# vladiant/CascadeClassifier

Measured on AMD Instinct MI355X. Metric: detection Mwindows/sec (1080p, haarcascade_frontalface) + achieved HBM GB/s, higher is better.
Workload: dtype i32+f32 (f64 stage sums)

## Files before the change

### cascadeclassifier_amd/_lib.py

```python
from __future__ import annotations

import ctypes as C
import os

_HERE = os.path.dirname(os.path.abspath(__file__))
LIB_PATH = os.environ.get("CCAMD_LIB") or os.path.join(_HERE, "lib", "libcascadeclassifier_amd.so")

CC_OK = 0
CC_ERR_INVALID_ARG = -1
CC_ERR_NO_DEVICE = -2
CC_ERR_HIP = -3
CC_ERR_IO = -4
CC_ERR_PARSE = -5
CC_ERR_UNSUPPORTED = -6
CC_ERR_BUFFER_TOO_SMALL = -7
CC_ERR_OUT_OF_RANGE = -8

CC_FEATURE_HAAR, CC_FEATURE_LBP, CC_FEATURE_HOG = 0, 1, 2
CC_PIX_GRAY8, CC_PIX_BGR8, CC_PIX_BGRA8, CC_PIX_RGB8, CC_PIX_RGBA8, CC_PIX_RGB8_PLANAR = 0, 1, 2, 3, 4, 5
CC_HAAR_BASIC, CC_HAAR_CORE, CC_HAAR_ALL = 0, 1, 2


class CascadeError(RuntimeError):

# ... 86 lines not shown
                                              _vp, C.POINTER(_i)]),
    "cc_detect_multiscale_levels_fmt": (_i, [_vp, _vp, _i, _i, _sz, _i, C.POINTER(DetectParams), _vp, _vp, _vp, _i,
                                             C.POINTER(_i)]),
    "cc_to_gray_u8": (_i, [_i, _vp, _i, _i, _i, _sz, _vp, _sz]),
    "cc_detect_multiscale_levels": (_i, [_vp, _vp, _i, _i, _sz, C.POINTER(DetectParams), _vp, _vp, _vp, _i, C.POINTER(_i)]),
    "cc_detect_raw": (_i, [_vp, _vp, _i, _i, _sz, C.POINTER(DetectParams), _vp, _i, C.POINTER(_i)]),
    "cc_detect_debug_windows": (_i, [_vp, _vp, _i, _i, _sz, C.POINTER(DetectParams), _vp, _vp, _vp, C.c_int64,
                                     C.POINTER(C.c_int64)]),
    "cc_scale_plan": (_i, [_i, _i, _i, _i, C.POINTER(DetectParams), _vp, _i, C.POINTER(_i)]),
    "cc_detector_specialize": (_i, [_vp, _i]),
    "cc_detector_specialize_async": (_i, [_vp, _i]),
    "cc_detector_specialized_stages": (_i, [_vp]),
    "cc_cascade_compile_specialized": (_i, [_vp, _i, C.c_char_p, C.POINTER(C.c_size_t)]),
    "cc_detector_set_profiling": (_i, [_vp, _i]),
    "cc_detector_graph_active": (_i, [_vp]),
    "cc_detector_graph_captures": (C.c_int64, [_vp]),
    "cc_detector_get_timings": (_i, [_vp, C.POINTER(DetectorTimings), _i]),
    "cc_detector_candidate_capacity": (_i, [_vp]),
    "cc_integral_u8": (_i, [_i, _vp, _i, _i, _sz, _vp, _vp, _vp]),
    "cc_resize_linear_exact_u8": (_i, [_i, _vp, _i, _i, _sz, _vp, _i, _i, _sz]),
    "cc_debug_stream_dwords": (_i, [_i, _sz, _i, C.POINTER(C.c_uint32)]),
    "cc_debug_division_check": (_i, [_i, C.c_uint64, C.c_uint64, C.POINTER(C.c_uint64)]),
    "cc_debug_vnf_check": (_i, [_i, C.c_uint64, C.c_uint64, C.POINTER(C.c_uint64)]),
    "cc_group_rectangles": (_i, [_vp, _i, _i, _d, _vp, _i, C.POINTER(_i)]),
    "cc_group_rectangles_device": (_i, [_i, _vp, _vp, _i, _i, _d, _vp, _i, _vp, C.POINTER(_i)]),
    "cc_group_rectangles_levels": (_i, [_vp, _vp, _vp, _i, _i, _d, _vp, _vp, _vp, _i, C.POINTER(_i)]),
    "cc_group_rectangles_device_levels": (_i, [_i, _vp, _vp, _vp, _vp, _i, _i, _d, _vp, _vp, _vp, _i, _vp, C.POINTER(_i)]),
    "cc_eval_create": (_i, [_i, _i, _i, _i, _i, _i, _pp]),
    "cc_eval_destroy": (None, [_vp]),
    "cc_eval_num_features": (_i, [_vp]),
    "cc_eval_max_cat_count": (_i, [_vp]),
    "cc_eval_feature_size": (_i, [_vp]),
    "cc_eval_feature_geometry": (_i, [_vp, _i, _vp, _vp, C.POINTER(_i)]),
    "cc_eval_set_image": (_i, [_vp, _vp, _sz, C.c_uint8, _i]),
    "cc_eval_set_images": (_i, [_vp, _vp, _i, _i, _vp]),
    "cc_eval_labels": (C.POINTER(C.c_float), [_vp]),
    "cc_eval_calc": (_i, [_vp, _i, _i, C.POINTER(C.c_float)]),
    "cc_eval_calc_list": (_i, [_vp, _vp, _i, _i, _vp]),
    "cc_eval_calc_batch": (_i, [_vp, _i, _i, _vp, _i, _vp, _i]),
    "cc_eval_calc_batch_device": (_i, [_vp, _i, _i, _vp, _i, _vp, _sz]),
    "cc_eval_calc_batch_sorted": (_i, [_vp, _i, _i, _i, _vp, _vp, _i]),
    "cc_eval_calc_custom_haar": (_i, [_vp, _vp, _i, _i, _vp, _i, _vp]),
    "cc_haar_feature_calc": (_i, [_i, _vp, _i, _i, _vp, _vp, _i, _i, _vp]),
    "cc_eval_get_sample": (_i, [_vp, _i, _vp, _vp, _vp]),
    "cc_eval_hog_feature_geometry": (_i, [_vp, _i, _vp]),
    "cc_eval_get_hog_sample": (_i, [_vp, _i, _vp, _vp]),
# ... 70 lines not shown
```

### cascadeclassifier_amd/csrc/cc_detect.hip

```cpp
#include <hip/hip_runtime.h>

#include <algorithm>

#include "cc_detector.h"

namespace ccamd {

#include "cc_eval_kernel.inc"

__global__ __launch_bounds__(256) void k_stream_dwords(const uint32_t* __restrict__ p, size_t n_words, uint32_t* __restrict__ out) {
  uint32_t acc = 0;
  for (size_t i = (size_t)blockIdx.x * blockDim.x + threadIdx.x; i < n_words; i += (size_t)gridDim.x * blockDim.x) acc += p[i];
  if (acc == 0x9e3779b9u) atomicAdd(out, acc);
  atomicAdd(out + 1 + (threadIdx.x & 15), acc);
}

__device__ __forceinline__ bool visited_by_scan(const unsigned long long* __restrict__ row_mask, int gx) {
  int run = 0;
  int pos = gx - 1;
  while (pos >= 0) {
    const int b = pos & 63;
    const unsigned long long w = row_mask[pos >> 6] << (63 - b);
    const int ones = min(__clzll((long long)~w), b + 1);
    run += ones;
// ... 82 lines not shown
  A.stage_first = d->d_stage_first.p;
  A.stage_ntrees = d->d_stage_ntrees.p;
  A.group_first = d->d_group_first.p;
  A.ngroups = d->n_groups;
  A.dense_from = d->dense_from;
  A.wave_below = d->wave_below;
  A.stop_after = d->stop_after;
  A.split_stumps = d->split_stumps;
  A.early_skip = d->early_skip;
  A.sq_compact = sq_compact;
  A.stage_thr = d->d_stage_thr.p;
  A.masks = d->d_masks[slot].p;
  A.mask_frame_words = P->mask_frame_words;
  A.cands = d->d_cands[slot].p;
  A.cand_count = d->d_counts[slot].p;
  A.cand_cap = d->cand_cap;
  A.stamps = nullptr;
  A.dbg_codes = debug ? d->d_dbg_codes.p : nullptr;
  A.dbg_sums = debug ? d->d_dbg_sums.p : nullptr;
  A.stumps1 = haar ? (const void*)d->d_haar1.p : (const void*)d->d_lbp1.p;
  A.stumps2 = haar ? (const void*)d->d_haar2.p : (const void*)d->d_lbp2.p;
  A.wstumps1 = d->d_haar1w.p ? (const void*)d->d_haar1w.p : A.stumps1;
  A.wstumps2 = d->d_haar2w.p ? (const void*)d->d_haar2w.p : A.stumps2;
  A.gstumps = haar ? (const void*)d->d_haar_g.p : (const void*)d->d_lbp_g.p;
  A.lbp16_all = d->lbp16_all;
  if (!haar && d->d_lbp16.p) A.wstumps2 = d->d_lbp16.p;
  A.trees = d->m.max_nodes_per_tree > 1 ? 1 : 0;
  A.nodes1 = haar ? (const void*)d->d_hnode1.p : (const void*)d->d_lnode1.p;
  A.nodes2 = haar ? (const void*)d->d_hnode2.p : (const void*)d->d_lnode2.p;
  A.tree_root = d->d_tree_root.p;
  A.tree_leaf0 = d->d_tree_leaf0.p;
  A.leaves = d->d_leaves.p;
  return A;
}

int eval_stamp_slots() { return STAMP_SLOTS; }

cc_status launch_eval(cc_detector* d, const Plan* P, int slot, int nchan, bool tilt, int sq_compact, bool debug, unsigned long long* stamps,
                      const EvalLaunch* launches, int n_launches, int nf, hipStream_t st) {
  const bool haar = d->m.feature_type == CC_FEATURE_HAAR;
  EvalArgs A = eval_args(d, P, slot, nchan, tilt, sq_compact, debug);
  A.stamps = stamps;
  for (int i = 0; i < n_launches; i++) {
    const EvalLaunch& L = launches[i];
    if (L.n_tiles == 0) continue;
    A.tiles = L.tiles;
// ... 79 lines not shown
```

### cascadeclassifier_amd/csrc/cc_detector.h

```cpp
#pragma once
#include <atomic>
#include <functional>
#include <future>
#include <map>
#include <memory>
#include <thread>

#include "cc_detect_internal.h"

namespace ccamd {

struct Plan {
  int w = 0, h = 0;
  cc_detect_params p{};
  std::vector<ScaleGeom> geom;
  FrontTables front;
  size_t mask_frame_words = 0;
  long long windows = 0, integral_elems = 0;
  int n_grid_rows = 0;
  struct TileList {
    int n = 0;
    DevBuf<int4> d;
  };
  std::map<std::pair<int, int>, TileList> tiles;
// ... 58 lines not shown

constexpr int kStageSlots = 3;

struct cc_detector {
  Cascade m;
  unsigned long long serial = 0;
  int device = 0;
  int max_batch = 1;
  int pass_capacity = 1;
  OwnStream own_stream;
  hipStream_t stream = nullptr;
  DevBuf<int> d_stage_ntrees, d_stage_first;
  std::vector<int> group_first;
  DevBuf<int> d_group_first;
  int n_groups = 0;
  int dense_from = 0x7fffffff;
  DevBuf<float> d_stage_thr;
  int wave_below = 0;
  int last_call_graph = 0;
  int stop_after = -1;
  int split_stumps = 0;
  DevBuf<HaarStumpDev> d_haar1, d_haar2;
  DevBuf<HaarStumpDev> d_haar1w, d_haar2w;
  DevBuf<HaarStumpDev> d_haar_g;
  DevBuf<LbpStumpDev> d_lbp_g, d_lbp16;
  int lbp16_all = 0;
  DevBuf<LbpStumpDev> d_lbp1, d_lbp2;
  DevBuf<HaarNodeDev> d_hnode1, d_hnode2;
  DevBuf<LbpNodeDev> d_lnode1, d_lnode2;
  DevBuf<int> d_tree_root, d_tree_leaf0;
  DevBuf<float> d_leaves;
  size_t lds = 0;
  std::vector<std::unique_ptr<Plan>> plans;
  DevBuf<uint8_t> d_frames, d_pyr;
  DevBuf<int32_t> d_integ[2], d_hbuf, d_diag, d_tseg;
  OwnStream front_stream;
  OwnEvent front_done[2], eval_done[2], batch_begin;
  bool eval_pending[2] = {false, false};
  int overlap_front = 1;
  SpecModule spec[2];
  int n_spec = 0;
  int last_stamp_tiles = 0;
  int spec_stages = 0;
  int auto_specialize = 0;
  std::thread spec_thread;
  std::atomic<int> spec_bg_state{0};
// ... 99 lines not shown
```

### cascadeclassifier_amd/csrc/cc_eval_kernel.inc

```

#define CC_CONST __attribute__((address_space(4)))
template <class T>
__device__ __forceinline__ const T CC_CONST* as_const_table(const T* p) {
  return (const T CC_CONST*)p;
}
template <class T>
__device__ __forceinline__ T load_record(const T CC_CONST* p) {
  static_assert(sizeof(T) % 4 == 0, "table records are dword multiples");
  T out;
  const int CC_CONST* w = (const int CC_CONST*)p;
  int* o = reinterpret_cast<int*>(&out);
#pragma unroll
  for (unsigned i = 0; i < sizeof(T) / 4; i++) o[i] = w[i];
  return out;
}

constexpr int STAGE_ROWS = 12;
template <int STEP, class Geom>
__device__ __forceinline__ void stage_tile(int32_t* lds, const Geom& G, const int32_t* __restrict__ sum,
                                           const ScaleDev& S, int x0, int y0) {
  const int lane = threadIdx.x & 63, wave = __builtin_amdgcn_readfirstlane(threadIdx.x >> 6);
  const int quads = (G.cols + 3) >> 2;
  const bool right_edge = x0 + quads * 4 - 1 > S.w;
  for (int q0 = 0; q0 < quads; q0 += 64) {
// ... 34 lines not shown
    }
  }
}

struct EvalArgs {
  const int32_t* integ;
  size_t int_frame_elems;
  int nchan;
  int tilt_chan;
  const ScaleDev* sd;
  const int4* tiles;
  int W0, H0;
  int nstages;
  const int* stage_first;
  const int* stage_ntrees;
  const float* stage_thr;
  const int* group_first;
  int ngroups;
  int dense_from;
  const void* stumps1;
  const void* stumps2;
  const void* wstumps1;
  const void* wstumps2;
  const void* gstumps;
  int lbp16_all;
  int trees;
  const void* nodes1;
  const void* nodes2;
  const int* tree_root;
  const int* tree_leaf0;
  const float* leaves;
  int wave_below;
  int early_skip;
  int sq_compact;
  int split_stumps;
  int stop_after;
  unsigned long long* masks;
  size_t mask_frame_words;
  CandRaw* cands;
  int* cand_count;
  int cand_cap;
  int32_t* dbg_codes;
  double* dbg_sums;
  unsigned long long* stamps;
};
constexpr int STAMP_SLOTS = 40;

struct LdsReader {
  const int32_t* b;
  __device__ __forceinline__ int operator()(int ofs) const { return b[ofs]; }
};
struct GlobalReader {
  const int32_t* g;
  unsigned org;
  int pitch;
  __device__ __forceinline__ int operator()(int p) const { return g[org + (unsigned)((p >> 16) * pitch + (p & 0xffff))]; }
};
template <class R>
__device__ __forceinline__ double stump_vote(const R& rd, const HaarStumpDev& sp, float vnf) {
  const int r0 = rd(sp.ofs[0][0]) - rd(sp.ofs[0][1]) - rd(sp.ofs[0][2]) + rd(sp.ofs[0][3]);
  const int r1 = rd(sp.ofs[1][0]) - rd(sp.ofs[1][1]) - rd(sp.ofs[1][2]) + rd(sp.ofs[1][3]);
  float v = sp.w[0] * (float)r0 + sp.w[1] * (float)r1;
  if (sp.nrect == 3) {
    const int r2 = rd(sp.ofs[2][0]) - rd(sp.ofs[2][1]) - rd(sp.ofs[2][2]) + rd(sp.ofs[2][3]);
    v += sp.w[2] * (float)r2;
  }
  v *= vnf;
  return (double)(v < sp.thr ? sp.left : sp.right);
}
template <class R>
__device__ __forceinline__ double stump_vote(const R& rd, const HaarStumpDev CC_CONST* spp, float vnf) {
  return stump_vote(rd, load_record(spp), vnf);
}

struct Lds16Reader {
  const unsigned short* h;
  __device__ __forceinline__ int operator()(int ofs) const { return (int)h[ofs]; }
};
template <bool M16, class R>
__device__ __forceinline__ float lbp_vote_f(const R& rd, const LbpStumpDev& sp) {
  int p[16];
#pragma unroll
  for (int j = 0; j < 16; j++) p[j] = rd(sp.ofs[j]);
  auto cell = [&](int a, int b, int c2, int d) {
    const int v = p[a] - p[b] - p[c2] + p[d];
    return M16 ? (v & 0xffff) : v;
  };
  const int c = cell(5, 6, 9, 10);
  const bool b7 = cell(0, 1, 4, 5) >= c, b6 = cell(1, 2, 5, 6) >= c, b5 = cell(2, 3, 6, 7) >= c;
  const int lo = (cell(6, 7, 10, 11) >= c ? 16 : 0) | (cell(10, 11, 14, 15) >= c ? 8 : 0) | (cell(9, 10, 13, 14) >= c ? 4 : 0) |
                 (cell(8, 9, 12, 13) >= c ? 2 : 0) | (cell(4, 5, 8, 9) >= c ? 1 : 0);
// ... 52 lines not shown

template <int CTRL, int ROW_MASK>
__device__ __forceinline__ int dpp_i32(int v) {
  return __builtin_amdgcn_update_dpp(0, v, CTRL, ROW_MASK, 0xF, false);
}
__device__ __forceinline__ int wave_max_u32(int v) {
  v = max(v, dpp_i32<0xB1, 0xF>(v));
  v = max(v, dpp_i32<0x4E, 0xF>(v));
  v = max(v, dpp_i32<0x141, 0xF>(v));
  v = max(v, dpp_i32<0x140, 0xF>(v));
  v = max(v, dpp_i32<0x142, 0xA>(v));
  v = max(v, dpp_i32<0x143, 0xC>(v));
  return __builtin_amdgcn_readlane(v, 63);
}
__device__ __forceinline__ int wave_sum_u32(int v) {
  v += dpp_i32<0xB1, 0xF>(v);
  v += dpp_i32<0x4E, 0xF>(v);
  v += dpp_i32<0x141, 0xF>(v);
  v += dpp_i32<0x140, 0xF>(v);
  v += dpp_i32<0x142, 0xA>(v);
  v += dpp_i32<0x143, 0xC>(v);
  return __builtin_amdgcn_readlane(v, 63);
}

__device__ __forceinline__ float inv_sqrt_as_float(double nf) {
#ifndef CC_EXACT_SLOW_VNF
  double y = __builtin_amdgcn_rsq(nf);
#pragma unroll
  for (int it = 0; it < 2; it++) {
    const double e = __builtin_fma(-(nf * y), y, 1.0);
    y = __builtin_fma(0.5 * y, e, y);
  }
  const unsigned below = (unsigned)(unsigned long long)__double_as_longlong(y) & 0x1fffffffu;
  if (__builtin_expect(below - 0x0ffffc00u > 0x800u, 1)) return (float)y;
#endif
  return (float)(1. / sqrt(nf));
}

#ifdef CC_SPEC_STAGES
template <int STEP>
__device__ __forceinline__ double spec_stage(int st, int p_lo, int p_hi, const int32_t* b, float vnf);
template <int STEP>
__device__ __forceinline__ void spec_stage0_x2(const int32_t* ba, const int32_t* bb, float vnfa, float vnfb, double& acc_a, double& acc_b);
#endif

template <bool C, class A, class B>
// ... 32 lines not shown
  const ScaleDev& S;
#ifdef CC_SPEC_W0
  static constexpr int W0 = CC_SPEC_W0, H0 = CC_SPEC_H0;
#else
  const int W0 = A.W0, H0 = A.H0;
#endif
  const Geom G{W0, H0};
  double* const s_part = reinterpret_cast<double*>(lds + tile_words_padded(G.words()) * ((HAAR && A.tilt_chan >= 0) ? 2 : 1));
  float* const s_vnf = reinterpret_cast<float*>(s_part + PART_DOUBLES);
  unsigned short* const s_q = reinterpret_cast<unsigned short*>(s_vnf + (HAAR ? TILE_Y * VNF_PITCH : 0));
  int* const s_cnt = reinterpret_cast<int*>(s_q + 2 * TILE_WINDOWS);
  const int frame = blockIdx.y;
  const int32_t* const sum = A.integ + ((size_t)frame * A.nchan + 0) * A.int_frame_elems + S.int_ofs;
  const int lane = threadIdx.x & 63, wave = __builtin_amdgcn_readfirstlane(threadIdx.x >> 6);
  const int half = lane >> 5, cls = lane & 31;
  const int gx0 = T.y * TILE_X, gy0 = T.z * TILE_Y;
  const int skew = (STEP * G.row_stride) & 31;
  const Node* const nodes = reinterpret_cast<const Node*>(STEP == 2 ? A.nodes2 : A.nodes1);
  const Stump CC_CONST* const stumps = as_const_table(reinterpret_cast<const Stump*>(G16 ? A.gstumps : STEP == 2 ? A.stumps2 : A.stumps1));
  const int CC_CONST* const stage_first = as_const_table(A.stage_first);
  const int CC_CONST* const stage_ntrees = as_const_table(A.stage_ntrees);
  const float CC_CONST* const stage_thr = as_const_table(A.stage_thr);
  const int CC_CONST* const group_first = as_const_table(A.group_first);
  const bool dbg = A.dbg_codes != nullptr && frame == 0;

  __device__ __forceinline__ EvalTile(const EvalArgs& A_, int32_t* lds_, const int4 T_, const ScaleDev& S_) : A(A_), lds(lds_), T(T_), S(S_) {}

  __device__ __forceinline__ void stamp(int slot) const {
    if (A.stamps && threadIdx.x == 0)
      A.stamps[((size_t)blockIdx.y * gridDim.x + blockIdx.x) * STAMP_SLOTS + slot] = __builtin_amdgcn_s_memtime();
  }
  __device__ __forceinline__ int window_base(int id) const { return ((id >> 6) * STEP) * G.row_stride + (id & 63); }
  __device__ __forceinline__ auto table_reader(int id) const {
    if constexpr (G16)
      return GlobalReader{sum, (unsigned)((gy0 + (id >> 6)) * STEP) * (unsigned)S.pitchI + (unsigned)((gx0 + (id & 63)) * STEP), S.pitchI};
    else
      return LdsReader{lds + window_base(id)};
  }
  __device__ __forceinline__ void report(int id, int code, double last) const {
    const size_t o = (size_t)S.win_ofs + (size_t)(gy0 + (id >> 6)) * S.nx + (gx0 + (id & 63));
    A.dbg_codes[o] = code;
    if (A.dbg_sums) A.dbg_sums[o] = last;
  }
  __device__ __forceinline__ void emit_candidate(int id, double last_sum) const {
    const int slot = atomicAdd(A.cand_count, 1);
    if (slot < A.cand_cap) A.cands[slot] = CandRaw{frame, T.x, gx0 + (id & 63), gy0 + (id >> 6), last_sum};
// ... 327 lines not shown
    const bool valid = row < h.my_rows;
    const int id = valid ? q[min(row, QUEUE_ROWS - 1) * 32 + cls] : cls;
    double acc = 0.;
    if (grp < rem) {
      [[maybe_unused]] const int32_t* b = lds + window_base(id);
      const float vnf = HAAR ? s_vnf[vnf_slot(id)] : 1.f;
#ifdef CC_SPEC_STAGES
      if (!TREES && st < CC_SPEC_STAGES)
        acc = spec_stage<STEP>(st, slice * (SPEC_PARTS / ns), (slice + 1) * (SPEC_PARTS / ns), b, vnf);
      else
#endif
        acc = table_sum(table_reader(id), first, nt, slice, ns, vnf);
      if (slice) s_part[(slice - 1) * (EVAL_THREADS / ns) + i] = acc;
    }
    __syncthreads();
    if (grp < rem && slice == 0) {
      for (int k = 1; k < ns; k++) acc += s_part[(k - 1) * (EVAL_THREADS / ns) + i];
      const bool pass = valid && !(acc < (double)stage_thr[st]);
      if (dbg && valid && !pass) report(id, -st, acc);
      deliver(pass, id, acc, last_group, h.qg + 1);
    }
  }

  __device__ __forceinline__ void wave_phase_haar(const QueueState& h) const {
    const int st = h.st;
    const Stump* wstumps = reinterpret_cast<const Stump*>(G16 ? A.gstumps : STEP == 2 ? A.wstumps2 : A.wstumps1);
    const WaveShare w = deal_windows(h);
    const int cnt = w.cnt, my_id = w.my_id;
    unsigned long long alive = w.alive;
    const bool w_stamps = st + 2 < 30;
    if (w_stamps) stamp(30);
    double tot = 0., last = 0.;
    int rej = 0;
    int s2 = st;
    for (; s2 < A.nstages && alive; s2++) {
      if (A.stop_after >= 0 && s2 > A.stop_after) break;
      const int first = stage_first[s2], nt = stage_ntrees[s2];
      for (int c = 0; c < nt; c += 64) {
        const int j = c + lane;
        const Stump rec = wstumps[first + min(j, nt - 1)];
        for (unsigned long long m = alive; m; m &= m - 1ull) {
          const int k = __builtin_ctzll(m);
          const int id = __builtin_amdgcn_readlane(my_id, k);
          const float vnf = s_vnf[vnf_slot(id)];
          const double part = j < nt ? stump_vote(table_reader(id), rec, vnf) : 0.;
          const double total = wave_sum_f64(part);
          if (lane == k) tot += total;
        }
      }
      const bool mine = (alive >> lane) & 1ull;
      const bool pass = mine && !(tot < (double)stage_thr[s2]);
      if (mine) {
        last = tot;
        if (!pass) rej = s2;
      }
      tot = 0.;
      alive = __ballot(pass);
      if (w_stamps && s2 - st < 8) stamp(31 + s2 - st);
    }
    const bool accepted = s2 == A.nstages && ((alive >> lane) & 1ull);
    if (lane < cnt) {
      if (accepted) emit_candidate(my_id, last);
      if (dbg && (accepted || !((alive >> lane) & 1ull))) report(my_id, accepted ? 1 : -rej, last);
    }
  }
  __device__ __forceinline__ void wave_phase_lbp(const QueueState& h) const {
    float* votes = reinterpret_cast<float*>(reinterpret_cast<char*>(s_part) + EVAL_WAVES * 128) + wave * 64;
    const WaveShare w = deal_windows(h);
    const int cnt = w.cnt, my_id = w.my_id;
    unsigned long long alive = w.alive;
    if (h.st + 2 < 30) stamp(30);
    const bool use16 = G16 && A.lbp16_all;
    const Stump* tab = reinterpret_cast<const Stump*>(G16 ? (use16 ? A.wstumps2 : A.gstumps) : STEP == 2 ? A.stumps2 : A.stumps1);
    double last = 0.;
    int code = 1;
    int s2 = h.st;
    while (s2 < A.nstages && alive) {
      if (A.stop_after >= 0 && s2 > A.stop_after) break;
      const int first = stage_first[s2];
// ... 117 lines not shown
```

### cascadeclassifier_amd/csrc/cc_host.cpp

```cpp
#include <algorithm>
#include <cfloat>
#include <cmath>
#include <cstdint>
#include <cstring>
#include <numeric>

#include "cc_internal.h"

namespace ccamd {

static thread_local std::string g_last_error;

cc_status set_error(cc_status code, const char* fmt, ...) {
  char buf[1024];
  va_list ap;
  va_start(ap, fmt);
  vsnprintf(buf, sizeof(buf), fmt, ap);
  va_end(ap);
  g_last_error = buf;
  return code;
}

static inline int rnd_f(float v) { return (int)std::nearbyintf(v); }
static inline int rnd_d(double v) { return (int)std::nearbyint(v); }
// ... 136 lines not shown
    const double q = std::ldexp(1.0, emin - 24);
    if (mag * headroom / q >= 9007199254740992.0) return false;
  }
  return true;
}

bool stage_quantum(const Cascade& m, int s, double& q) {
  int emin = INT32_MAX;
  double mag = 0;
  for (int i = 0; i < m.stage_ntrees[(size_t)s]; i++) {
    const size_t k = (size_t)m.stage_first[(size_t)s] + i;
    const float l = m.stump_left[k], r = m.stump_right[k];
    mag += std::max(std::fabs((double)l), std::fabs((double)r));
    for (float v : {l, r})
      if (v != 0.0f) {
        int e;
        std::frexp(v, &e);
        emin = std::min(emin, e);
      }
  }
  if (emin == INT32_MAX) return false;
  q = std::ldexp(1.0, emin - 24);
  return mag / q < 2147483647.0;
}

void group_rectangles(std::vector<cc_rect>& rects, int group_threshold, double eps, std::vector<int>* levels,
                      std::vector<double>* level_weights) {
  const int n = (int)rects.size();
  if (group_threshold <= 0 || n == 0) return;
  std::vector<int> parent(n), rank_(n, 0);
  std::iota(parent.begin(), parent.end(), 0);
  auto find = [&](int a) {
    int r = a;
    while (parent[r] != r) r = parent[r];
    while (parent[a] != r) {
      int nx = parent[a];
      parent[a] = r;
      a = nx;
    }
    return r;
  };
  std::vector<int> order(n);
  std::iota(order.begin(), order.end(), 0);
  std::sort(order.begin(), order.end(), [&](int a, int b) { return rects[a].x < rects[b].x; });
  for (int oi = 0; oi < n; oi++) {
    const int i = order[oi];
// ... 299 lines not shown
```

### cascadeclassifier_amd/csrc/cc_internal.h

```cpp
#pragma once

#include <cstdarg>
#include <cstdint>
#include <cstdio>
#include <string>
#include <vector>

#include "../../include/cascadeclassifier_amd.h"

#include <locale.h>

namespace ccamd {

struct CNumericLocale {
  locale_t prev = (locale_t)0;
  CNumericLocale() {
    static locale_t c = newlocale(LC_ALL_MASK, "C", (locale_t)0);
    if (c != (locale_t)0) prev = uselocale(c);
  }
  ~CNumericLocale() {
    if (prev != (locale_t)0) uselocale(prev);
  }
  CNumericLocale(const CNumericLocale&) = delete;
  CNumericLocale& operator=(const CNumericLocale&) = delete;
// ... 49 lines not shown
cc_status cascade_from_xml(const XmlNode& root, Cascade& out);

struct ScaleGeom {
  float scale;
  int w, h, ystep, nx, ny, win_w, win_h;
};
void scale_plan(int W0, int H0, int imgw, int imgh, const cc_detect_params& p, std::vector<ScaleGeom>& out);

struct AxisTaps {
  std::vector<int32_t> ofs;
  std::vector<uint16_t> w1;
};
void linear_exact_taps(int src, int dst, AxisTaps& t);

void group_rectangles(std::vector<cc_rect>& rects, int group_threshold, double eps, std::vector<int>* levels = nullptr,
                      std::vector<double>* level_weights = nullptr);

std::vector<int> pass_sizes(int n_frames, int max_batch, int pipeline_passes, bool pipeline_passes_set, bool want_results,
                            bool defer_last);

void stage_groups(const std::vector<int32_t>& stage_ntrees, int from, int budget, int dense_stage, std::vector<int>& group_first,
                  int& dense_from);

void haar_catalog(int W, int H, int mode, std::vector<HaarFeature>& out);
void lbp_catalog(int W, int H, std::vector<int32_t>& rects);
void hog_catalog(int W, int H, std::vector<int32_t>& blocks);

struct CatSplit {
  bool found;
  double quality;
  int n_left;
  int32_t subset[8];
};
void split_categories(const double* hist, int n_cat, bool is_classifier, bool gini, CatSplit& out);

}

struct cc_cascade {
  ccamd::Cascade m;
};
```

### cascadeclassifier_amd/csrc/cc_tables.hip

```cpp
#include <algorithm>
#include <cstdlib>

#include "cc_detector.h"

namespace ccamd {

static std::vector<HaarStumpDev> schedule_for_wave_phase(const Cascade& m, const std::vector<HaarStumpDev>& t) {
  std::vector<HaarStumpDev> out;
  out.reserve(t.size());
  auto variant = [](const HaarStumpDev& s, int v) {
    HaarStumpDev r = s;
    for (int j = 0; j < 3; j++) {
      if (v & (1 << (2 * j))) std::swap(r.ofs[j][0], r.ofs[j][3]);
      if (v & (2 << (2 * j))) std::swap(r.ofs[j][1], r.ofs[j][2]);
    }
    return r;
  };
  for (size_t s = 0; s < m.stage_ntrees.size(); s++) {
    const int first = m.stage_first[s], nt = m.stage_ntrees[s];
    std::vector<char> used((size_t)nt, 0);
    int left = nt;
    while (left > 0) {
      std::vector<std::vector<int>> words(12 * 32);
      int mx[12] = {0};
// ... 21 lines not shown
              best_v = v;
              if (cost == 0) break;
            }
          }
          if (best_cost == 0) break;
        }
        const HaarStumpDev r = variant(t[(size_t)first + best], best_v);
        const int nslots = r.nrect == 3 ? 12 : 8;
        for (int k = 0; k < nslots; k++) {
          const int o = r.ofs[k >> 2][k & 3];
          std::vector<int>& w = words[(size_t)k * 32 + (o & 31)];
          if (std::find(w.begin(), w.end(), o) == w.end()) w.push_back(o);
          mx[k] = std::max(mx[k], (int)w.size());
        }
        out.push_back(r);
        used[(size_t)best] = 1;
        left--;
      }
    }
  }
  return out;
}

template <int STEP>
static void build_haar_nodes(const Cascade& m, std::vector<HaarNodeDev>& out) {
  const TileGeom<STEP> G(m.win_w, m.win_h);
  out.resize(m.node_feature.size());
  for (size_t i = 0; i < out.size(); i++) {
    HaarNodeDev& d = out[i];
    std::memset(&d, 0, sizeof(d));
    fill_haar_corners(m, m.node_feature[i], d, [&](int y, int x) { return G.at(y, x); }, tile_words_padded(G.words()));
    d.thr = m.node_threshold[i];
    d.left = m.node_left[i];
    d.right = m.node_right[i];
  }
}
template <int STEP>
static void build_lbp_nodes(const Cascade& m, std::vector<LbpNodeDev>& out) {
  const TileGeom<STEP> G(m.win_w, m.win_h);
  out.resize(m.node_feature.size());
  for (size_t i = 0; i < out.size(); i++) {
    LbpNodeDev& d = out[i];
    std::memset(&d, 0, sizeof(d));
    fill_lbp_cells(m, m.node_feature[i], i, d, [&](int y, int x) { return G.at(y, x); });
    d.left = m.node_left[i];
    d.right = m.node_right[i];
// ... 8 lines not shown
  const bool haar = d->m.feature_type == CC_FEATURE_HAAR;
  const TileGeom<1> G1(d->m.win_w, d->m.win_h);
  const TileGeom<2> G2(d->m.win_w, d->m.win_h);
  d->lds = eval_lds_bytes(std::max(G1.words(), G2.words()), d->m.has_tilted, haar);
  const bool trees = d->m.max_nodes_per_tree > 1;
  const bool exact = !trees && stage_sums_order_independent(d->m);
  d->wave_below = (haar && exact) ? 24 : 0;
  if (!haar && !trees) {
    bool fits = true;
    for (int v : d->m.stage_ntrees) fits = fits && v <= 64;
    d->wave_below = fits ? 24 : 0;
  }
  d->split_stumps = exact ? 1 : 0;
  if (const char* e = std::getenv("CCAMD_SPLIT_STUMPS")) d->split_stumps = d->split_stumps && std::atoi(e) != 0;
  if (const char* e = std::getenv("CCAMD_DEBUG_STOP_AFTER_STAGE")) d->stop_after = std::atoi(e);
  d->early_skip = std::getenv("CCAMD_NO_EARLY_SKIP") ? 0 : 1;
  if (const char* e = std::getenv("CCAMD_PIPELINE_PASSES")) {
    d->pipeline_passes = std::max(1, std::atoi(e));
    d->pipeline_passes_set = 1;
  }
  if (const char* e = std::getenv("CCAMD_CAND_CAP")) d->cand_cap = std::max(16, std::atoi(e));
  if (const char* e = std::getenv("CCAMD_WAVE_BELOW"))
    if (d->wave_below) d->wave_below = std::max(0, std::min(64, std::atoi(e)));
  const bool lbp = !haar && !trees;
  int budget = lbp ? 14 : 0;
  const int from = lbp ? 2 : 1;
  if (const char* e = std::getenv("CCAMD_GROUP_STUMPS")) budget = trees ? 0 : std::max(0, std::atoi(e));
  int dense_stage = lbp ? 2 : -1;
  if (const char* e = std::getenv("CCAMD_DENSE_FROM")) dense_stage = std::atoi(e);
  stage_groups(d->m.stage_ntrees, from, budget, dense_stage, d->group_first, d->dense_from);
  d->n_groups = (int)d->group_first.size() - 1;
  if (const char* e = std::getenv("CCAMD_AUTO_SPECIALIZE")) d->auto_specialize = std::atoi(e);
}

cc_status upload_cascade_tables(cc_detector* d) {
  const bool haar = d->m.feature_type == CC_FEATURE_HAAR;
  const bool trees = d->m.max_nodes_per_tree > 1;
  CC_HIP(d->d_stage_ntrees.upload(d->m.stage_ntrees, d->stream));
  CC_HIP(d->d_stage_first.upload(d->m.stage_first, d->stream));
  CC_HIP(d->d_stage_thr.upload(d->m.stage_threshold, d->stream));
  CC_HIP(d->d_group_first.upload(d->group_first, d->stream));
  CC_HIP(hipStreamSynchronize(d->stream));
  if (trees) {
    std::vector<int> root(d->m.tree_first_node.begin(), d->m.tree_first_node.end()), leaf0(d->m.tree_first_leaf.begin(), d->m.tree_first_leaf.end());
    CC_HIP(d->d_tree_root.upload(root, d->stream));
    CC_HIP(d->d_tree_leaf0.upload(leaf0, d->stream));
// ... 4 lines not shown
      build_haar_nodes<2>(d->m, n2);
      CC_HIP(d->d_hnode1.upload(n1, d->stream));
      CC_HIP(d->d_hnode2.upload(n2, d->stream));
      CC_HIP(hipStreamSynchronize(d->stream));
    } else {
      std::vector<LbpNodeDev> n1, n2;
      build_lbp_nodes<1>(d->m, n1);
      build_lbp_nodes<2>(d->m, n2);
      CC_HIP(d->d_lnode1.upload(n1, d->stream));
      CC_HIP(d->d_lnode2.upload(n2, d->stream));
      CC_HIP(hipStreamSynchronize(d->stream));
    }
  } else if (haar) {
    std::vector<HaarStumpDev> s1, s2;
    build_haar_stumps<1>(d->m, s1);
    build_haar_stumps<2>(d->m, s2);
    CC_HIP(d->d_haar1.upload(s1, d->stream));
    CC_HIP(d->d_haar2.upload(s2, d->stream));
    std::vector<HaarStumpDev> sg;
    if (!d->m.has_tilted) build_haar_gstumps(d->m, sg);
    CC_HIP(d->d_haar_g.upload(sg, d->stream));
    CC_HIP(hipStreamSynchronize(d->stream));
    if (d->wave_below > 0) {
      const std::vector<HaarStumpDev> w1 = schedule_for_wave_phase(d->m, s1), w2 = schedule_for_wave_phase(d->m, s2);
      CC_HIP(d->d_haar1w.upload(w1, d->stream));
      CC_HIP(d->d_haar2w.upload(w2, d->stream));
      CC_HIP(hipStreamSynchronize(d->stream));
    }
  } else {
    std::vector<LbpStumpDev> s1, s2;
    build_lbp_stumps<1>(d->m, s1);
    build_lbp_stumps<2>(d->m, s2);
    CC_HIP(d->d_lbp1.upload(s1, d->stream));
    CC_HIP(d->d_lbp2.upload(s2, d->stream));
    std::vector<LbpStumpDev> sg, s16;
    build_lbp_gstumps(d->m, sg);
    CC_HIP(d->d_lbp_g.upload(sg, d->stream));
    d->lbp16_all = 1;
    for (size_t i = 0; i < d->m.stump_feature.size(); i++) {
      const int32_t* r = &d->m.lbp_rects[(size_t)d->m.stump_feature[i] * 4];
      if (!fits16((long long)r[2] * r[3])) d->lbp16_all = 0;
    }
    if (d->lbp16_all) {
      build_lbp_stumps16(d->m, s16);
      CC_HIP(d->d_lbp16.upload(s16, d->stream));
    }
    CC_HIP(hipStreamSynchronize(d->stream));
  }
  return CC_OK;
}

}
```

### cascadeclassifier_amd/detector.py

```python
from __future__ import annotations

import ctypes as C
from dataclasses import dataclass

import numpy as np

from . import _lib as L


def _params(scale_factor, min_neighbors, min_size, max_size) -> L.DetectParams:
    mn = min_size or (0, 0)
    mx = max_size or (0, 0)
    return L.DetectParams(float(scale_factor), int(min_neighbors), int(mn[0]), int(mn[1]), int(mx[0]), int(mx[1]))


def _vp(a):
    return None if a is None else a.ctypes.data_as(C.c_void_p)


def _view(ptr, ctype, n):
    if not ptr or n == 0:
        return np.zeros(0, np.dtype(ctype))
    return np.ctypeslib.as_array(C.cast(ptr, C.POINTER(ctype)), shape=(n,)).copy()

# ... 210 lines not shown
        a, b, c = C.c_void_p(), C.c_void_p(), C.c_void_p()
        L.check(L.lib().cc_cascade_stages(self._c, C.byref(a), C.byref(b), C.byref(c)))
        ns, nw, nf = inf["n_stages"], inf["n_weak"], inf["n_features"]
        sf, sn, sthr = _view(a, C.c_int32, ns), _view(b, C.c_int32, ns), _view(c, C.c_float, ns)
        stump = [None] * 5
        if inf["max_nodes_per_tree"] == 1:
            p = [C.c_void_p() for _ in range(5)]
            L.check(L.lib().cc_cascade_stumps(self._c, *[C.byref(x) for x in p]))
            stump = [_view(p[0], C.c_int32, nw), _view(p[1], C.c_float, nw), _view(p[2], C.c_float, nw),
                     _view(p[3], C.c_float, nw),
                     _view(p[4], C.c_int32, nw * inf["subset_size"]).reshape(nw, -1) if inf["subset_size"] else None]
        r, w, t = C.c_void_p(), C.c_void_p(), C.c_void_p()
        L.check(L.lib().cc_cascade_features(self._c, C.byref(r), C.byref(w), C.byref(t)))
        if inf["feature_type"] == L.CC_FEATURE_HAAR:
            rects = _view(r, C.c_int32, nf * 12).reshape(nf, 3, 4)
            weights = _view(w, C.c_float, nf * 3).reshape(nf, 3)
            tilted = _view(t, C.c_int32, nf)
        elif inf["feature_type"] == L.CC_FEATURE_HOG:
            rects, weights, tilted = _view(r, C.c_int32, nf * 5).reshape(nf, 5), None, None
        else:
            rects, weights, tilted = _view(r, C.c_int32, nf * 4).reshape(nf, 4), None, None
        return CascadeModel(inf, sf, sn, sthr, *stump, rects, weights, tilted)

    def _detector(self):
        if not self._c:
            raise L.CascadeError(L.CC_ERR_INVALID_ARG, "CascadeClassifier is empty")
        if not self._d:
            L.check(L.lib().cc_detector_create(self._c, self.device, self.max_batch, C.byref(self._d)))
        return self._d

    def set_stream(self, hip_stream: int | None):
        L.check(L.lib().cc_detector_set_stream(self._detector(), C.c_void_p(hip_stream or 0)))

    def detectMultiScale(self, image, scaleFactor=1.1, minNeighbors=3, flags=0, minSize=None, maxSize=None,
                         pixel_format=None) -> np.ndarray:
        image = np.ascontiguousarray(image, np.uint8)
        _, h, w, fmt, rs, _ = frame_layout(image.shape, pixel_format)
        p = _params(scaleFactor, minNeighbors, minSize, maxSize)
        cap = 1024
        while True:
            out = np.zeros((cap, 4), np.int32)
            n = C.c_int(0)
            st = L.lib().cc_detect_multiscale_fmt(self._detector(), _vp(image), w, h, rs, fmt, C.byref(p), _vp(out), cap,
                                                  C.byref(n))
            if st == L.CC_ERR_BUFFER_TOO_SMALL:
                cap = n.value
# ... 219 lines not shown
```

### include/cascadeclassifier_amd.h

```cpp
#ifndef CASCADECLASSIFIER_AMD_H_
#define CASCADECLASSIFIER_AMD_H_

#include <stddef.h>
#include <stdint.h>

#ifdef __cplusplus
extern "C" {
#endif

#if defined(__GNUC__)
#define CC_API __attribute__((visibility("default")))
#else
#define CC_API
#endif

typedef int cc_status;
enum {
  CC_OK = 0,
  CC_ERR_INVALID_ARG = -1,
  CC_ERR_NO_DEVICE = -2,
  CC_ERR_HIP = -3,
  CC_ERR_IO = -4,
  CC_ERR_PARSE = -5,
  CC_ERR_UNSUPPORTED = -6,
// ... 134 lines not shown
  int64_t resize_launches, integral_launches, eval_launches, finalize_launches;
  int64_t frames;
  int64_t grid_windows;
  int64_t integral_elems;
  double eval_step1_ms;
  double group_ms;
  int64_t group_launches;
} cc_detector_timings;
CC_API cc_status cc_detector_set_profiling(cc_detector* d, int enabled);
CC_API int cc_detector_candidate_capacity(const cc_detector* d);
CC_API cc_status cc_detector_get_timings(cc_detector* d, cc_detector_timings* t, int reset);
CC_API int cc_detector_graph_active(const cc_detector* d);
CC_API int64_t cc_detector_graph_captures(const cc_detector* d);

CC_API cc_status cc_integral_u8(int device, const uint8_t* img, int width, int height, size_t row_stride, int32_t* sum,
                                int32_t* sqsum, int32_t* tilted);
CC_API cc_status cc_resize_linear_exact_u8(int device, const uint8_t* src, int sw, int sh, size_t sstride, uint8_t* dst,
                                           int dw, int dh, size_t dstride);
CC_API cc_status cc_to_gray_u8(int device, const uint8_t* src, int pixel_format, int width, int height, size_t row_stride,
                               uint8_t* dst, size_t dst_stride);
CC_API cc_status cc_debug_stream_dwords(int device, size_t n_bytes, int repeats, uint32_t* checksum);
CC_API cc_status cc_debug_division_check(int device, uint64_t n_pairs, uint64_t seed, uint64_t* mismatches);
CC_API cc_status cc_debug_vnf_check(int device, uint64_t n_values, uint64_t seed, uint64_t* mismatches);
CC_API cc_status cc_group_rectangles(const cc_rect* rects, int n, int group_threshold, double eps, cc_rect* out, int cap,
                                     int* n_out);
CC_API cc_status cc_group_rectangles_device(int device, const cc_rect* rects, const int32_t* offsets, int n_frames,
                                            int group_threshold, double eps, cc_rect* out, int cap, int32_t* out_offsets,
                                            int* n_total);
CC_API cc_status cc_group_rectangles_levels(const cc_rect* rects, const int32_t* levels, const double* weights, int n,
                                            int group_threshold, double eps, cc_rect* out, int32_t* out_levels,
                                            double* out_weights, int cap, int* n_out);
CC_API cc_status cc_group_rectangles_device_levels(int device, const cc_rect* rects, const int32_t* levels,
                                                   const double* weights, const int32_t* offsets, int n_frames,
                                                   int group_threshold, double eps, cc_rect* out, int32_t* out_levels,
                                                   double* out_weights, int cap, int32_t* out_offsets, int* n_total);

typedef struct cc_evaluator cc_evaluator;
enum { CC_HAAR_BASIC = 0, CC_HAAR_CORE = 1, CC_HAAR_ALL = 2 };

CC_API cc_status cc_eval_create(int feature_type, int haar_mode, int win_w, int win_h, int max_samples, int device,
                                cc_evaluator** out);
CC_API void cc_eval_destroy(cc_evaluator* e);
CC_API int cc_eval_num_features(const cc_evaluator* e);
CC_API int cc_eval_max_cat_count(const cc_evaluator* e);
CC_API int cc_eval_feature_size(const cc_evaluator* e);
CC_API cc_status cc_eval_feature_geometry(const cc_evaluator* e, int fi, int32_t* rects, float* weights, int* tilted);
// ... 101 lines not shown
```

Baseline: 19070.

## Use exact integer stage sums in wave phase for quantizable Haar stages

```diff
diff --git a/cascadeclassifier_amd/_lib.py b/cascadeclassifier_amd/_lib.py
--- a/cascadeclassifier_amd/_lib.py
+++ b/cascadeclassifier_amd/_lib.py
@@ -132,6 +132,7 @@
     "cc_debug_stream_dwords": (_i, [_i, _sz, _i, C.POINTER(C.c_uint32)]),
     "cc_debug_division_check": (_i, [_i, C.c_uint64, C.c_uint64, C.POINTER(C.c_uint64)]),
     "cc_debug_vnf_check": (_i, [_i, C.c_uint64, C.c_uint64, C.POINTER(C.c_uint64)]),
+    "cc_debug_wave_int_tables": (_i, [_vp, _vp, _vp, _vp, _vp]),
     "cc_group_rectangles": (_i, [_vp, _i, _i, _d, _vp, _i, C.POINTER(_i)]),
     "cc_group_rectangles_device": (_i, [_i, _vp, _vp, _i, _i, _d, _vp, _i, _vp, C.POINTER(_i)]),
     "cc_group_rectangles_levels": (_i, [_vp, _vp, _vp, _i, _i, _d, _vp, _vp, _vp, _i, C.POINTER(_i)]),
diff --git a/cascadeclassifier_amd/csrc/cc_detect.hip b/cascadeclassifier_amd/csrc/cc_detect.hip
--- a/cascadeclassifier_amd/csrc/cc_detect.hip
+++ b/cascadeclassifier_amd/csrc/cc_detect.hip
@@ -128,6 +128,8 @@
   A.stumps2 = haar ? (const void*)d->d_haar2.p : (const void*)d->d_lbp2.p;
   A.wstumps1 = d->d_haar1w.p ? (const void*)d->d_haar1w.p : A.stumps1;
   A.wstumps2 = d->d_haar2w.p ? (const void*)d->d_haar2w.p : A.stumps2;
+  A.wave_q = d->d_wave_q.p;
+  A.wave_thr_q = d->d_wave_thr_q.p;
   A.gstumps = haar ? (const void*)d->d_haar_g.p : (const void*)d->d_lbp_g.p;
   A.lbp16_all = d->lbp16_all;
   if (!haar && d->d_lbp16.p) A.wstumps2 = d->d_lbp16.p;
diff --git a/cascadeclassifier_amd/csrc/cc_detector.h b/cascadeclassifier_amd/csrc/cc_detector.h
--- a/cascadeclassifier_amd/csrc/cc_detector.h
+++ b/cascadeclassifier_amd/csrc/cc_detector.h
@@ -104,6 +104,10 @@
   int split_stumps = 0;
   DevBuf<HaarStumpDev> d_haar1, d_haar2;
   DevBuf<HaarStumpDev> d_haar1w, d_haar2w;
+  int wave_int_enabled = 1;
+  WaveIntTables wave_int;
+  DevBuf<double> d_wave_q;
+  DevBuf<int> d_wave_thr_q;
   DevBuf<HaarStumpDev> d_haar_g;
   DevBuf<LbpStumpDev> d_lbp_g, d_lbp16;
   int lbp16_all = 0;
diff --git a/cascadeclassifier_amd/csrc/cc_eval_kernel.inc b/cascadeclassifier_amd/csrc/cc_eval_kernel.inc
--- a/cascadeclassifier_amd/csrc/cc_eval_kernel.inc
+++ b/cascadeclassifier_amd/csrc/cc_eval_kernel.inc
@@ -80,6 +80,8 @@
   const void* stumps2;
   const void* wstumps1;
   const void* wstumps2;
+  const double* wave_q;
+  const int* wave_thr_q;
   const void* gstumps;
   int lbp16_all;
   int trees;
@@ -115,7 +117,7 @@
   __device__ __forceinline__ int operator()(int p) const { return g[org + (unsigned)((p >> 16) * pitch + (p & 0xffff))]; }
 };
 template <class R>
-__device__ __forceinline__ double stump_vote(const R& rd, const HaarStumpDev& sp, float vnf) {
+__device__ __forceinline__ bool stump_goes_left(const R& rd, const HaarStumpDev& sp, float vnf) {
   const int r0 = rd(sp.ofs[0][0]) - rd(sp.ofs[0][1]) - rd(sp.ofs[0][2]) + rd(sp.ofs[0][3]);
   const int r1 = rd(sp.ofs[1][0]) - rd(sp.ofs[1][1]) - rd(sp.ofs[1][2]) + rd(sp.ofs[1][3]);
   float v = sp.w[0] * (float)r0 + sp.w[1] * (float)r1;
@@ -124,7 +126,18 @@
     v += sp.w[2] * (float)r2;
   }
   v *= vnf;
-  return (double)(v < sp.thr ? sp.left : sp.right);
+  return v < sp.thr;
+}
+template <class R>
+__device__ __forceinline__ double stump_vote(const R& rd, const HaarStumpDev& sp, float vnf) {
+  return (double)(stump_goes_left(rd, sp, vnf) ? sp.left : sp.right);
+}
+template <class Acc, class R>
+__device__ __forceinline__ Acc stump_vote_as(const R& rd, const HaarStumpDev& sp, float vnf) {
+  if constexpr (sizeof(Acc) == sizeof(int))
+    return stump_goes_left(rd, sp, vnf) ? __float_as_int(sp.left) : __float_as_int(sp.right);
+  else
+    return stump_vote(rd, sp, vnf);
 }
 template <class R>
 __device__ __forceinline__ double stump_vote(const R& rd, const HaarStumpDev CC_CONST* spp, float vnf) {
@@ -223,6 +236,8 @@
   v += dpp_i32<0x143, 0xC>(v);
   return __builtin_amdgcn_readlane(v, 63);
 }
+__device__ __forceinline__ int wave_total(int v) { return wave_sum_u32(v); }
+__device__ __forceinline__ double wave_total(double v) { return wave_sum_f64(v); }
 
 __device__ __forceinline__ float inv_sqrt_as_float(double nf) {
 #ifndef CC_EXACT_SLOW_VNF
@@ -301,6 +316,8 @@
   const int CC_CONST* const stage_ntrees = as_const_table(A.stage_ntrees);
   const float CC_CONST* const stage_thr = as_const_table(A.stage_thr);
   const int CC_CONST* const group_first = as_const_table(A.group_first);
+  const double CC_CONST* const wave_q = as_const_table(A.wave_q);
+  const int CC_CONST* const wave_thr_q = as_const_table(A.wave_thr_q);
   const bool dbg = A.dbg_codes != nullptr && frame == 0;
 
   __device__ __forceinline__ EvalTile(const EvalArgs& A_, int32_t* lds_, const int4 T_, const ScaleDev& S_) : A(A_), lds(lds_), T(T_), S(S_) {}
@@ -674,6 +691,24 @@
     }
   }
 
+  template <class Acc>
+  __device__ __forceinline__ Acc wave_stage(const Stump* wstumps, int s2, unsigned long long alive, int my_id) const {
+    const int first = stage_first[s2], nt = stage_ntrees[s2];
+    Acc tot = 0;
+    for (int c = 0; c < nt; c += 64) {
+      const int j = c + lane;
+      const Stump rec = wstumps[first + min(j, nt - 1)];
+      for (unsigned long long m = alive; m; m &= m - 1ull) {
+        const int k = __builtin_ctzll(m);
+        const int id = __builtin_amdgcn_readlane(my_id, k);
+        const float vnf = s_vnf[vnf_slot(id)];
+        const Acc part = j < nt ? stump_vote_as<Acc>(table_reader(id), rec, vnf) : Acc(0);
+        const Acc total = wave_total(part);
+        if (lane == k) tot += total;
+      }
+    }
+    return tot;
+  }
   __device__ __forceinline__ void wave_phase_haar(const QueueState& h) const {
     const int st = h.st;
     const Stump* wstumps = reinterpret_cast<const Stump*>(G16 ? A.gstumps : STEP == 2 ? A.wstumps2 : A.wstumps1);
@@ -682,31 +717,28 @@
     unsigned long long alive = w.alive;
     const bool w_stamps = st + 2 < 30;
     if (w_stamps) stamp(30);
-    double tot = 0., last = 0.;
+    double last = 0.;
     int rej = 0;
     int s2 = st;
     for (; s2 < A.nstages && alive; s2++) {
       if (A.stop_after >= 0 && s2 > A.stop_after) break;
-      const int first = stage_first[s2], nt = stage_ntrees[s2];
-      for (int c = 0; c < nt; c += 64) {
-        const int j = c + lane;
-        const Stump rec = wstumps[first + min(j, nt - 1)];
-        for (unsigned long long m = alive; m; m &= m - 1ull) {
-          const int k = __builtin_ctzll(m);
-          const int id = __builtin_amdgcn_readlane(my_id, k);
-          const float vnf = s_vnf[vnf_slot(id)];
-          const double part = j < nt ? stump_vote(table_reader(id), rec, vnf) : 0.;
-          const double total = wave_sum_f64(part);
-          if (lane == k) tot += total;
-        }
+      const double q = G16 ? 0. : wave_q[s2];
+      double tot;
+      bool at_least_thr;
+      if (q != 0.) {
+        const int n = wave_stage<int>(wstumps, s2, alive, my_id);
+        tot = (double)n * q;
+        at_least_thr = n >= wave_thr_q[s2];
+      } else {
+        tot = wave_stage<double>(wstumps, s2, alive, my_id);
+        at_least_thr = !(tot < (double)stage_thr[s2]);
       }
       const bool mine = (alive >> lane) & 1ull;
-      const bool pass = mine && !(tot < (double)stage_thr[s2]);
+      const bool pass = mine && at_least_thr;
       if (mine) {
         last = tot;
         if (!pass) rej = s2;
       }
-      tot = 0.;
       alive = __ballot(pass);
       if (w_stamps && s2 - st < 8) stamp(31 + s2 - st);
     }
diff --git a/cascadeclassifier_amd/csrc/cc_host.cpp b/cascadeclassifier_amd/csrc/cc_host.cpp
--- a/cascadeclassifier_amd/csrc/cc_host.cpp
+++ b/cascadeclassifier_amd/csrc/cc_host.cpp
@@ -182,6 +182,30 @@
   if (emin == INT32_MAX) return false;
   q = std::ldexp(1.0, emin - 24);
   return mag / q < 2147483647.0;
+}
+
+WaveIntTables wave_int_tables(const Cascade& m, bool enabled) {
+  const size_t ns = m.stage_ntrees.size();
+  WaveIntTables t;
+  t.q.assign(ns, 0.0);
+  t.thr_q.assign(ns, 0);
+  t.left_q.assign(m.stump_left.size(), 0);
+  t.right_q.assign(m.stump_left.size(), 0);
+  if (!enabled || m.feature_type != CC_FEATURE_HAAR || m.max_nodes_per_tree != 1 || !stage_sums_order_independent(m, 1.0)) return t;
+  for (size_t s = 0; s < ns; s++) {
+    double q;
+    const double thr = (double)m.stage_threshold[s];
+    if (std::isnan(thr) || !stage_quantum(m, (int)s, q)) continue;
+    const double x = std::ceil(thr / q);
+    t.q[s] = q;
+    t.thr_q[s] = x >= 2147483647.0 ? INT32_MAX : x <= -2147483648.0 ? INT32_MIN : (int32_t)x;
+    for (int i = 0; i < m.stage_ntrees[s]; i++) {
+      const size_t k = (size_t)m.stage_first[s] + i;
+      t.left_q[k] = (int32_t)((double)m.stump_left[k] / q);
+      t.right_q[k] = (int32_t)((double)m.stump_right[k] / q);
+    }
+  }
+  return t;
 }
 
 void group_rectangles(std::vector<cc_rect>& rects, int group_threshold, double eps, std::vector<int>* levels,
diff --git a/cascadeclassifier_amd/csrc/cc_internal.h b/cascadeclassifier_amd/csrc/cc_internal.h
--- a/cascadeclassifier_amd/csrc/cc_internal.h
+++ b/cascadeclassifier_amd/csrc/cc_internal.h
@@ -95,6 +95,13 @@
 void stage_groups(const std::vector<int32_t>& stage_ntrees, int from, int budget, int dense_stage, std::vector<int>& group_first,
                   int& dense_from);
 
+struct WaveIntTables {
+  std::vector<double> q;
+  std::vector<int32_t> thr_q;
+  std::vector<int32_t> left_q, right_q;
+};
+WaveIntTables wave_int_tables(const Cascade& m, bool enabled);
+
 void haar_catalog(int W, int H, int mode, std::vector<HaarFeature>& out);
 void lbp_catalog(int W, int H, std::vector<int32_t>& rects);
 void hog_catalog(int W, int H, std::vector<int32_t>& blocks);
diff --git a/cascadeclassifier_amd/csrc/cc_tables.hip b/cascadeclassifier_amd/csrc/cc_tables.hip
--- a/cascadeclassifier_amd/csrc/cc_tables.hip
+++ b/cascadeclassifier_amd/csrc/cc_tables.hip
@@ -67,6 +67,22 @@
   return out;
 }
 
+static void put_integer_leaves(const Cascade& m, const WaveIntTables& t, std::vector<HaarStumpDev>& w) {
+  for (size_t s = 0; s < m.stage_ntrees.size(); s++) {
+    if (t.q[s] == 0.0) continue;
+    for (int i = 0; i < m.stage_ntrees[s]; i++) {
+      HaarStumpDev& r = w[(size_t)m.stage_first[s] + i];
+      static_assert(sizeof(r.left) == sizeof(int32_t), "leaf words");
+      std::memcpy(&r.left, &t.left_q[(size_t)r.pad], sizeof(int32_t));
+      std::memcpy(&r.right, &t.right_q[(size_t)r.pad], sizeof(int32_t));
+    }
+  }
+}
+static bool wave_int_wanted() {
+  const char* e = std::getenv("CCAMD_WAVE_INT");
+  return !e || std::atoi(e) != 0;
+}
+
 template <int STEP>
 static void build_haar_nodes(const Cascade& m, std::vector<HaarNodeDev>& out) {
   const TileGeom<STEP> G(m.win_w, m.win_h);
@@ -121,6 +137,8 @@
   if (const char* e = std::getenv("CCAMD_CAND_CAP")) d->cand_cap = std::max(16, std::atoi(e));
   if (const char* e = std::getenv("CCAMD_WAVE_BELOW"))
     if (d->wave_below) d->wave_below = std::max(0, std::min(64, std::atoi(e)));
+  d->wave_int_enabled = wave_int_wanted();
+  d->wave_int = wave_int_tables(d->m, d->wave_int_enabled && haar && d->wave_below > 0);
   const bool lbp = !haar && !trees;
   int budget = lbp ? 14 : 0;
   const int from = lbp ? 2 : 1;
@@ -171,9 +189,13 @@
     CC_HIP(d->d_haar_g.upload(sg, d->stream));
     CC_HIP(hipStreamSynchronize(d->stream));
     if (d->wave_below > 0) {
-      const std::vector<HaarStumpDev> w1 = schedule_for_wave_phase(d->m, s1), w2 = schedule_for_wave_phase(d->m, s2);
+      std::vector<HaarStumpDev> w1 = schedule_for_wave_phase(d->m, s1), w2 = schedule_for_wave_phase(d->m, s2);
+      put_integer_leaves(d->m, d->wave_int, w1);
+      put_integer_leaves(d->m, d->wave_int, w2);
       CC_HIP(d->d_haar1w.upload(w1, d->stream));
       CC_HIP(d->d_haar2w.upload(w2, d->stream));
+      CC_HIP(d->d_wave_q.upload(d->wave_int.q, d->stream));
+      CC_HIP(d->d_wave_thr_q.upload(d->wave_int.thr_q, d->stream));
       CC_HIP(hipStreamSynchronize(d->stream));
     }
   } else {
@@ -200,3 +222,13 @@
 }
 
 }
+
+extern "C" cc_status cc_debug_wave_int_tables(const cc_cascade* c, double* q, int32_t* thr_q, int32_t* left_q, int32_t* right_q) {
+  if (!c) return set_error(CC_ERR_INVALID_ARG, "cc_debug_wave_int_tables: null cascade");
+  const WaveIntTables t = wave_int_tables(c->m, wave_int_wanted());
+  if (q) std::copy(t.q.begin(), t.q.end(), q);
+  if (thr_q) std::copy(t.thr_q.begin(), t.thr_q.end(), thr_q);
+  if (left_q) std::copy(t.left_q.begin(), t.left_q.end(), left_q);
+  if (right_q) std::copy(t.right_q.begin(), t.right_q.end(), right_q);
+  return CC_OK;
+}
diff --git a/cascadeclassifier_amd/detector.py b/cascadeclassifier_amd/detector.py
--- a/cascadeclassifier_amd/detector.py
+++ b/cascadeclassifier_amd/detector.py
@@ -256,6 +256,13 @@
             rects, weights, tilted = _view(r, C.c_int32, nf * 4).reshape(nf, 4), None, None
         return CascadeModel(inf, sf, sn, sthr, *stump, rects, weights, tilted)
 
+    def wave_int_tables(self):
+        inf = self.info()
+        q, thr_q = np.zeros(inf["n_stages"], np.float64), np.zeros(inf["n_stages"], np.int32)
+        left_q, right_q = np.zeros(inf["n_weak"], np.int32), np.zeros(inf["n_weak"], np.int32)
+        L.check(L.lib().cc_debug_wave_int_tables(self._c, _vp(q), _vp(thr_q), _vp(left_q), _vp(right_q)))
+        return q, thr_q, left_q, right_q
+
     def _detector(self):
         if not self._c:
             raise L.CascadeError(L.CC_ERR_INVALID_ARG, "CascadeClassifier is empty")
diff --git a/include/cascadeclassifier_amd.h b/include/cascadeclassifier_amd.h
--- a/include/cascadeclassifier_amd.h
+++ b/include/cascadeclassifier_amd.h
@@ -180,6 +180,7 @@
 CC_API cc_status cc_debug_stream_dwords(int device, size_t n_bytes, int repeats, uint32_t* checksum);
 CC_API cc_status cc_debug_division_check(int device, uint64_t n_pairs, uint64_t seed, uint64_t* mismatches);
 CC_API cc_status cc_debug_vnf_check(int device, uint64_t n_values, uint64_t seed, uint64_t* mismatches);
+CC_API cc_status cc_debug_wave_int_tables(const cc_cascade* c, double* q, int32_t* thr_q, int32_t* left_q, int32_t* right_q);
 CC_API cc_status cc_group_rectangles(const cc_rect* rects, int n, int group_threshold, double eps, cc_rect* out, int cap,
                                      int* n_out);
 CC_API cc_status cc_group_rectangles_device(int device, const cc_rect* rects, const int32_t* offsets, int n_frames,
```

New measurement: 19260 (median of 6 runs). 1.01x the previous value.
